# mousecpn/Boosting-R-CNN

Hardware: AMD Instinct MI355X
Metric: images/sec (1333x800) Boosting R-CNN R50-PAFPN inference (higher is better)
Workload: dtype f32; 1 GPU; boosting_rcnn_r50_pafpn_1x_utdac.py inference (model(return_loss=False, rescale=True): device pass + result copy + bbox2result), batch 8 x 3x800x1344 per GPU, f32 MFMA conv stack, 1000 pre-NMS / 256 proposals per image, seeded synthetic weights; global_batch=8, parallelism=dp1

## Files before the change

### boosting-r-cnn_amd/csrc/conv_common.h

```cpp
#pragma once
#include "common.h"

namespace brcnn_conv {

typedef float f32x16 __attribute__((ext_vector_type(16)));
typedef float f32x4 __attribute__((ext_vector_type(4)));
typedef unsigned int u32x4 __attribute__((ext_vector_type(4)));

constexpr int OOB = 0x7fffffff;

constexpr int BK = 32, LDS_STRIDE = 36;

struct ConvParams {
    const float* x;
    const float* w;
    const float* scale;
    const float* shift;
    const float* residual;
    float* y;
    int batch, Cin, Cout, KH, KW, stride, pad;
    int M, K;
    int relu;
    int tiles_m, tiles_n;
    int pitch;
// ... 60 lines not shown
        const int qh = hi / dilate, qw = wi / dilate;
        ok = ok & (qh * dilate == hi) & (qw * dilate == wi);
        hi = qh;
        wi = qw;
    }
}

typedef short brcnn_i16x2 __attribute__((ext_vector_type(2)));
__device__ __forceinline__ float brcnn_relu1(float v) { return __builtin_amdgcn_fmed3f(v, 0.f, __builtin_inff()); }
template <int ET> __device__ __forceinline__ brcnn_f32x2 brcnn_unpk2(unsigned w) {
    brcnn_f32x2 r;
    if constexpr (ET) {
        r.x = brcnn_h2f((unsigned short)(w & 0xffffu));
        r.y = brcnn_h2f((unsigned short)(w >> 16));
    } else {
        r.x = __uint_as_float(w << 16);
        r.y = __uint_as_float(w & 0xffff0000u);
    }
    return r;
}
template <int ET> __device__ __forceinline__ unsigned brcnn_pk2(brcnn_f32x2 v) { return ET ? brcnn_pk2h(v.x, v.y) : brcnn_pk2b(v.x, v.y); }
__device__ __forceinline__ unsigned brcnn_relu_pk(unsigned w, unsigned floor2) {
    const brcnn_i16x2 a = __builtin_bit_cast(brcnn_i16x2, w), f = __builtin_bit_cast(brcnn_i16x2, floor2);
    return __builtin_bit_cast(unsigned, __builtin_elementwise_max(a, f));
}

int conv1x1_stream_try(ConvParams& p, hipStream_t s, int f16);
int conv1x1_stream_set(int mode);
int dispatch_conv_bf16(ConvParams& p, hipStream_t s);
int dispatch_conv_pp_bf16(ConvParams& p, hipStream_t s);
int dispatch_conv_pp128_bf16(ConvParams& p, hipStream_t s);
int sk_plan_pp(ConvParams& p, int slots, int bm, int bn, hipStream_t s);
int sk_plan_pp_f32(ConvParams& p, int slots, int bm, int bn, hipStream_t s);
float* conv_ws_wgrad_slabs(hipStream_t s);
float* wgrad_defer_slabs(hipStream_t s, size_t bytes, int* err);
void wgrad_defer_push(hipStream_t s, float* slab, float* dw, int tiles, int tiles_k, int slices, int group, int Cout, int K,
                      int kind);
unsigned* conv_ws_wgrad_counters(hipStream_t s);
int wgrad_pp_bf16_try(const void* x, const void* dy, void* dw, int batch, int num_segments, const int* heights_host,
                      const int* widths_host, int cin, int cout, int kh, int kw, int stride, int pad, hipStream_t stream,
                      int f16);
int wgrad_pp_set(int v);
bool sk_par_enabled();
int dispatch_conv_pp_f32(ConvParams& p, hipStream_t s);

}
```

### boosting-r-cnn_amd/csrc/conv_igemm.hip

```cpp
#include "conv_common.h"

namespace {
using namespace brcnn_conv;

template <bool FAST, int WM, int NT, bool RES>
__global__ __launch_bounds__(128 * WM, 2) void conv_igemm_f32_kernel(ConvParams p) {
    constexpr int THREADS = 128 * WM;
    constexpr int BM = 64 * WM, BN = 64 * NT;
    constexpr int RPP = THREADS / 8;
    constexpr int AJ = BM / RPP;
    constexpr int BJ = (BN + RPP - 1) / RPP;
    extern __shared__ __attribute__((aligned(16))) float smem[];
    float* As = smem;
    float* Bs = smem + 2 * BM * LDS_STRIDE;

    const int tid = threadIdx.x;
    const int lane = tid & 63, wave = tid >> 6;
    const int wm = wave >> 1, wn = wave & 1;
    const int li = lane & 31, lh = lane >> 5;
    const float* __restrict__ xin = p.x;

    const int nwg = p.tiles_m * p.tiles_n;
    const int tile = xcd_remap(blockIdx.x, nwg);
    const int tile_m = tile / p.tiles_n, tile_n = tile - tile_m * p.tiles_n;
// ... 175 lines not shown
        mfma_group(as, bs, 0);
        mfma_group(as, bs, 1);
        if (more) store_tile(cur ^ 1);
        mfma_group(as, bs, 2);
        mfma_group(as, bs, 3);
        __syncthreads();
        cur ^= 1;
    }

    float* __restrict__ yout = p.y;
#pragma unroll
    for (int tn = 0; tn < NT; tn++) {
        const int co = n0 + wn * 32 * NT + tn * 32 + li;
        const bool cok = co < p.Cout;
        const float sc = (p.scale && cok) ? p.scale[co] : 1.f;
        const float sh = (p.shift && cok) ? p.shift[co] : 0.f;
#pragma unroll
        for (int tm = 0; tm < 2; tm++) {
            const int mb = m0 + wm * 64 + tm * 32 + 4 * lh;
#pragma unroll
            for (int r = 0; r < 16; r++) {
                const int m = mb + (r & 3) + 8 * (r >> 2);
                float v = acc[tm][tn][r];
                if (p.scale) v = v * sc;
                v = v + sh;
                if (RES) v = v + rv[tm][tn][r];
                if (p.relu) v = fmaxf(v, 0.f);
                if (cok && m < p.M) yout[(size_t)m * p.Cout + co] = v;
            }
        }
    }
}

template <int MT, int NT, bool RES>
__global__ __launch_bounds__(256, 2) void conv_igemm_f32_dma_kernel(ConvParams p) {
    constexpr int BM = 64 * MT, BN = 64 * NT;
    constexpr int AG = BM / 8 / 4;
    constexpr int BG = BN / 8 / 4;
    extern __shared__ __attribute__((aligned(16))) float smem[];
    float* As = smem;
    float* Bs = smem + 2 * BM * 32;
    typedef __attribute__((address_space(3))) void* lds_ptr_t;

    const int tid = threadIdx.x;
    const int lane = tid & 63;
    const int wave = __builtin_amdgcn_readfirstlane(tid >> 6);
    const int wm = wave >> 1, wn = wave & 1;
    const int li = lane & 31, lh = lane >> 5;

    const int nwg = p.tiles_m * p.tiles_n;
    const int tile = xcd_remap(blockIdx.x, nwg);
    const int tile_m = tile / p.tiles_n, tile_n = tile - tile_m * p.tiles_n;
    const int m0 = tile_m * BM, n0 = tile_n * BN;

    const __amdgpu_buffer_rsrc_t rsrc_x = __builtin_amdgcn_make_buffer_rsrc((void*)p.x, 0, (int)p.x_bytes, 0x00020000);
    const __amdgpu_buffer_rsrc_t rsrc_w = __builtin_amdgcn_make_buffer_rsrc((void*)p.w, 0, (int)p.w_bytes, 0x00020000);

    const int rg = lane >> 3, pc = lane & 7;
    const bool plain = !p.no_fast && p.KH == 1 && p.KW == 1 && p.stride == 1 && p.pad == 0 && p.nseg == 1 && p.dilate <= 1;
    int a_base[AG], a_hw[AG], a_H[AG], a_W[AG], a_lc[AG];
    int b_off[BG];
#pragma unroll
    for (int j = 0; j < AG; j++) {
        const int r = (wave * AG + j) * 8 + rg;
        a_lc[j] = (pc ^ ((r >> 1) & 7)) * 4;
        const int m = m0 + r;
        if (plain) {
            a_base[j] = m < p.M ? (int)p.seg_xoff[0] + m * p.pitch : -1;
            a_hw[j] = (4096 << 16) | 4096;
            a_H[j] = a_W[j] = 1;
        } else if (m < p.M) {
            int sg = 0;
#pragma unroll
            for (int t = 1; t < BRCNN_MAX_LEVELS; t++)
                if (t < p.nseg && m >= p.seg_m0[t]) sg = t;
            const int ml = m - p.seg_m0[sg];
            const int Ho = p.seg_Ho[sg], Wo = p.seg_Wo[sg];
            a_H[j] = p.seg_H[sg];
            a_W[j] = p.seg_W[sg];
            const int n = ml / (Ho * Wo);
            const int rem = ml - n * (Ho * Wo);
            const int ho = rem / Wo, wo = rem - ho * Wo;
            a_base[j] = (int)p.seg_xoff[sg] + n * a_H[j] * a_W[j] * p.pitch;
            a_hw[j] = ((ho * p.stride - p.pad + 4096) << 16) | (wo * p.stride - p.pad + 4096);
        } else {
            a_base[j] = -1;
            a_hw[j] = 0;
            a_H[j] = a_W[j] = 0;
        }
    }
#pragma unroll
    for (int j = 0; j < BG; j++) {
        const int r = (wave * BG + j) * 8 + rg;
        const int co = n0 + r;
        b_off[j] = (co < p.Cout) ? co * p.K + (pc ^ ((r >> 1) & 7)) * 4 : -1;
    }

    f32x16 acc[MT][NT];
#pragma unroll
    for (int a = 0; a < MT; a++)
#pragma unroll
        for (int b = 0; b < NT; b++)
#pragma unroll
            for (int r = 0; r < 16; r++) acc[a][b][r] = 0.f;

    const int nk = (p.K + BK - 1) / BK;

    int d_k0 = 0, d_ci0 = 0, d_kh = 0, d_kw = 0;
    unsigned a_off4[AG], b_off4[BG];
#pragma unroll
    for (int j = 0; j < AG; j++) a_off4[j] = a_base[j] >= 0 ? (unsigned)(a_base[j] + a_lc[j] + tile_n * p.gstep) * 4u : (unsigned)OOB;
#pragma unroll
    for (int j = 0; j < BG; j++) b_off4[j] = b_off[j] >= 0 ? (unsigned)b_off[j] * 4u : (unsigned)OOB;
    unsigned d_plain = 0;
    auto dma_tile_plain = [&](int buf) {
        const unsigned step = d_plain;
        d_plain += BK * 4;
#pragma unroll
        for (int j = 0; j < AG; j++) {
            float* dst = As + buf * BM * 32 + (wave * AG + j) * 8 * 32;
            __builtin_amdgcn_raw_ptr_buffer_load_lds(rsrc_x, (lds_ptr_t)dst, 16, (int)(a_off4[j] + step), 0, 0, 0);
        }
#pragma unroll
        for (int j = 0; j < BG; j++) {
            float* dst = Bs + buf * BN * 32 + (wave * BG + j) * 8 * 32;
            __builtin_amdgcn_raw_ptr_buffer_load_lds(rsrc_w, (lds_ptr_t)dst, 16, (int)(b_off4[j] + step), 0, 0, 0);
        }
    };
    auto dma_tile = [&](int kt, int buf) {
        (void)kt;
        if (plain) { dma_tile_plain(buf); return; }
        const int ci0 = d_ci0, kh = d_kh, kw = d_kw;
        const int k0 = (kh * p.KW + kw) * p.Cin + ci0;
        (void)d_k0;
        if (++d_kw == p.KW) {
            d_kw = 0;
            if (++d_kh == p.KH) { d_kh = 0; d_ci0 += BK; }
        }
#pragma unroll
        for (int j = 0; j < AG; j++) {
            int hi = (a_hw[j] >> 16) - 4096 + kh;
            int wi = (a_hw[j] & 0xffff) - 4096 + kw;
            bool ok = a_base[j] >= 0;
            if (p.dilate > 1) {
                brcnn_undilate(p.dilate, hi, wi, ok);
            }
            ok = ok & ((unsigned)hi < (unsigned)a_H[j]) & ((unsigned)wi < (unsigned)a_W[j]);
            const int off = ok ? (a_base[j] + (hi * a_W[j] + wi) * p.pitch + ci0 + a_lc[j] + tile_n * p.gstep) * 4 : OOB;
            float* dst = As + buf * BM * 32 + (wave * AG + j) * 8 * 32;
            __builtin_amdgcn_raw_ptr_buffer_load_lds(rsrc_x, (lds_ptr_t)dst, 16, off, 0, 0, 0);
        }
#pragma unroll
        for (int j = 0; j < BG; j++) {
            const int off = (b_off[j] >= 0) ? (b_off[j] + k0) * 4 : OOB;
            float* dst = Bs + buf * BN * 32 + (wave * BG + j) * 8 * 32;
            __builtin_amdgcn_raw_ptr_buffer_load_lds(rsrc_w, (lds_ptr_t)dst, 16, off, 0, 0, 0);
        }
    };

    dma_tile(0, 0);

    const float* __restrict__ res = p.residual;
    const bool vec = (p.Cout & 3) == 0;
    const int vrow = lane >> 3, vcol = (lane & 7) * 4;
    float rv[MT][NT][16];
    const bool full = !p.no_fast && vec && !p.scatter && m0 + BM <= p.M && n0 + BN <= p.Cout;
    const size_t row0 = (size_t)(m0 + wm * 32 * MT + vrow) * p.Cout + n0 + wn * 32 * NT + vcol;
// ... 8 lines not shown
                    for (int it = 0; it < 4; it++) {
                        const float4 q = *reinterpret_cast<const float4*>(rrow + (size_t)(tm * 32 + it * 8) * p.Cout + tn * 32);
                        rv[tm][tn][4 * it + 0] = q.x; rv[tm][tn][4 * it + 1] = q.y;
                        rv[tm][tn][4 * it + 2] = q.z; rv[tm][tn][4 * it + 3] = q.w;
                    }
            return;
        }
#pragma unroll
        for (int tn = 0; tn < NT; tn++) {
#pragma unroll
            for (int tm = 0; tm < MT; tm++) {
                if (vec) {
                    const int co = n0 + wn * 32 * NT + tn * 32 + vcol;
#pragma unroll
                    for (int it = 0; it < 4; it++) {
                        const int m = m0 + wm * 32 * MT + tm * 32 + it * 8 + vrow;
                        float4 q = make_float4(0.f, 0.f, 0.f, 0.f);
                        if (co < p.Cout && m < p.M) q = *reinterpret_cast<const float4*>(res + (size_t)m * p.Cout + co);
                        rv[tm][tn][4 * it + 0] = q.x; rv[tm][tn][4 * it + 1] = q.y;
                        rv[tm][tn][4 * it + 2] = q.z; rv[tm][tn][4 * it + 3] = q.w;
                    }
                } else {
                    const int co = n0 + wn * 32 * NT + tn * 32 + li;
                    const int mb = m0 + wm * 32 * MT + tm * 32 + 4 * lh;
#pragma unroll
                    for (int r = 0; r < 16; r++) {
                        const int m = mb + (r & 3) + 8 * (r >> 2);
                        rv[tm][tn][r] = (co < p.Cout && m < p.M) ? res[(size_t)m * p.Cout + co] : 0.f;
                    }
                }
            }
        }
    };
    asm volatile("s_waitcnt vmcnt(0)" ::: "memory");
    __syncthreads();

    const int sw = (li >> 1) & 7;
    unsigned chb[BK / 8];
#pragma unroll
    for (int kk = 0; kk < BK / 8; kk++) chb[kk] = (unsigned)(((2 * kk + lh) ^ sw) * 16);
    const unsigned a_lane = (unsigned)(size_t)(lds_ptr_t)(As + (wm * 32 * MT + li) * 32);
    const unsigned b_lane = (unsigned)(size_t)(lds_ptr_t)(Bs + (wn * 32 * NT + li) * 32);
    f32x4 av[2][MT], bv[2][NT];
    auto frag_read = [&](int slot, unsigned a_addr, unsigned b_addr) {
        asm volatile("ds_read_b128 %0, %1" : "=v"(av[slot][0]) : "v"(a_addr) : "memory");
        if constexpr (MT == 2)
            asm volatile("ds_read_b128 %0, %1 offset:4096" : "=v"(av[slot][1]) : "v"(a_addr) : "memory");
        asm volatile("ds_read_b128 %0, %1" : "=v"(bv[slot][0]) : "v"(b_addr) : "memory");
        if constexpr (NT == 2)
            asm volatile("ds_read_b128 %0, %1 offset:4096" : "=v"(bv[slot][1]) : "v"(b_addr) : "memory");
    };
    auto frag_wait = [&](int slot) {
        if constexpr (MT == 2 && NT == 2)
            asm volatile("s_waitcnt lgkmcnt(0)" : "+v"(av[slot][0]), "+v"(av[slot][1]), "+v"(bv[slot][0]), "+v"(bv[slot][1]) :: "memory");
        else if constexpr (MT == 2)
            asm volatile("s_waitcnt lgkmcnt(0)" : "+v"(av[slot][0]), "+v"(av[slot][1]), "+v"(bv[slot][0]) :: "memory");
        else if constexpr (NT == 2)
            asm volatile("s_waitcnt lgkmcnt(0)" : "+v"(av[slot][0]), "+v"(bv[slot][0]), "+v"(bv[slot][1]) :: "memory");
        else
            asm volatile("s_waitcnt lgkmcnt(0)" : "+v"(av[slot][0]), "+v"(bv[slot][0]) :: "memory");
    };
    auto compute_tile = [&](int cur, bool prefetch) {
        const unsigned a_cur = a_lane + cur * (BM * 32 * 4);
        const unsigned b_cur = b_lane + cur * (BN * 32 * 4);
        __builtin_amdgcn_s_setprio(1);
        frag_read(0, a_cur + chb[0], b_cur + chb[0]);
        if (prefetch) dma_tile(0, cur ^ 1);
        frag_wait(0);
        __builtin_amdgcn_s_setprio(0);
#pragma unroll
        for (int kk = 0; kk < BK / 8; kk++) {
            const int sl = kk & 1;
            if (kk + 1 < BK / 8) frag_read(sl ^ 1, a_cur + chb[kk + 1], b_cur + chb[kk + 1]);
#pragma unroll
            for (int e = 0; e < 4; e++)
#pragma unroll
                for (int tm = 0; tm < MT; tm++)
#pragma unroll
                    for (int t = 0; t < NT; t++)
                        acc[tm][t] = __builtin_amdgcn_mfma_f32_32x32x2f32(av[sl][tm][e], bv[sl][t][e],
                                                                          acc[tm][t], 0, 0, 0);
            if (kk + 1 < BK / 8) frag_wait(sl ^ 1);
        }
    };
    int cur = 0;
    for (int kt = 0; kt + 1 < nk; kt++) {
        compute_tile(cur, true);
        asm volatile("s_waitcnt vmcnt(0)" ::: "memory");
        __syncthreads();
        cur ^= 1;
    }
    if (RES) load_residual();
    compute_tile(cur, false);

    float* __restrict__ yout = p.y;
    float* slab = (wave < 2 ? As + (cur ^ 1) * BM * 32 : Bs + (cur ^ 1) * BN * 32) + (wave & 1) * 1024;
    if (full) {
        float* __restrict__ yrow = yout + row0;
#pragma unroll
        for (int tn = 0; tn < NT; tn++) {
            const int co = n0 + wn * 32 * NT + tn * 32 + li;
            const float sc = p.scale ? p.scale[co] : 1.f;
            const float sh = p.shift ? p.shift[co] : 0.f;
#pragma unroll
            for (int tm = 0; tm < MT; tm++) {
#pragma unroll
                for (int r = 0; r < 16; r += 2) {
                    const brcnn_f32x2 a = brcnn_f32x2{acc[tm][tn][r], acc[tm][tn][r + 1]} * brcnn_f32x2{sc, sc} + brcnn_f32x2{sh, sh};
                    slab[((r & 3) + 8 * (r >> 2) + 4 * lh) * 32 + li] = a.x;
                    slab[(((r + 1) & 3) + 8 * ((r + 1) >> 2) + 4 * lh) * 32 + li] = a.y;
                }
                __builtin_amdgcn_wave_barrier();
#pragma unroll
                for (int it = 0; it < 4; it++) {
                    float4 v = *reinterpret_cast<const float4*>(slab + (it * 8 + vrow) * 32 + vcol);
                    if (RES) {
                        v.x += rv[tm][tn][4 * it + 0]; v.y += rv[tm][tn][4 * it + 1];
                        v.z += rv[tm][tn][4 * it + 2]; v.w += rv[tm][tn][4 * it + 3];
                    }
                    if (p.relu) {
                        v.x = brcnn_relu1(v.x); v.y = brcnn_relu1(v.y); v.z = brcnn_relu1(v.z); v.w = brcnn_relu1(v.w);
                    }
                    *reinterpret_cast<float4*>(yrow + (size_t)(tm * 32 + it * 8) * p.Cout + tn * 32) = v;
                }
                __builtin_amdgcn_wave_barrier();
            }
// ... 25 lines not shown
                    if (RES) {
                        v.x += rv[tm][tn][4 * it + 0]; v.y += rv[tm][tn][4 * it + 1];
                        v.z += rv[tm][tn][4 * it + 2]; v.w += rv[tm][tn][4 * it + 3];
                    }
                    if (p.relu) {
                        v.x = fmaxf(v.x, 0.f); v.y = fmaxf(v.y, 0.f); v.z = fmaxf(v.z, 0.f); v.w = fmaxf(v.w, 0.f);
                    }
                    if (cv < p.Cout && m < p.M) {
                        const long long ro = out_row_offset(p, m);
                        if (ro >= 0) *reinterpret_cast<float4*>(yout + ro + cv) = v;
                    }
                }
                __builtin_amdgcn_wave_barrier();
            } else {
                const int mb = m0 + wm * 32 * MT + tm * 32 + 4 * lh;
#pragma unroll
                for (int r = 0; r < 16; r++) {
                    const int m = mb + (r & 3) + 8 * (r >> 2);
                    float v = acc[tm][tn][r];
                    if (p.scale) v = v * sc;
                    v = v + sh;
                    if (RES) v = v + rv[tm][tn][r];
                    if (p.relu) v = fmaxf(v, 0.f);
                    if (cok && m < p.M) {
                        const long long ro = out_row_offset(p, m);
                        if (ro >= 0) yout[ro + co] = v;
                    }
                }
            }
        }
    }
}

template <int MT, int NT, bool RES>
int launch_dma(const ConvParams& p, hipStream_t s) {
    const size_t lds = (size_t)2 * (64 * MT + 64 * NT) * 32 * sizeof(float);
    static bool attr_done = false;
    if (!attr_done) {
        BRCNN_HIP_CHECK(hipFuncSetAttribute((const void*)conv_igemm_f32_dma_kernel<MT, NT, RES>,
                                            hipFuncAttributeMaxDynamicSharedMemorySize, (int)lds));
        attr_done = true;
    }
    hipLaunchKernelGGL((conv_igemm_f32_dma_kernel<MT, NT, RES>), dim3(p.tiles_m * p.tiles_n), dim3(256), lds,
                       s, p);
    BRCNN_LAUNCH_CHECK();
    return 0;
}

template <bool FAST, int WM, int NT, bool RES>
int launch_conv(const ConvParams& p, hipStream_t s) {
    const size_t lds = (size_t)2 * (64 * WM + 64 * NT) * LDS_STRIDE * sizeof(float);
    static bool attr_done = false;
    if (!attr_done) {
        BRCNN_HIP_CHECK(hipFuncSetAttribute((const void*)conv_igemm_f32_kernel<FAST, WM, NT, RES>,
                                            hipFuncAttributeMaxDynamicSharedMemorySize, (int)lds));
        attr_done = true;
    }
    hipLaunchKernelGGL((conv_igemm_f32_kernel<FAST, WM, NT, RES>), dim3(p.tiles_m * p.tiles_n),
                       dim3(128 * WM), lds, s, p);
    BRCNN_LAUNCH_CHECK();
    return 0;
}

template <bool FAST, int WM, int NT>
int launch_res(const ConvParams& p, hipStream_t s) {
    return p.residual ? launch_conv<FAST, WM, NT, true>(p, s) : launch_conv<FAST, WM, NT, false>(p, s);
}

int g_use_dma = 1;
int g_force_wm = 0, g_force_nt = 0;

int g_no_fast = 0;
int g_pp_f32_n128 = 1;
int g_pp_f32_mode = 1;

int dispatch_conv(ConvParams& p, hipStream_t s) {
    const bool fast = (p.Cin % 32 == 0);
    if (fast && g_pp_f32_mode && g_force_wm == 0 && g_force_nt == 0 && !p.gstep && (p.Cout % 256) == 0 && p.K >= 256 &&
        p.KH * p.KW <= 32 && !(p.dilate > 1 && p.residual)) {
        const long long t48 = (long long)((p.M + 127) / 128) * (p.Cout / 256);
        p.pp_rows = g_pp_f32_mode >= 128 ? g_pp_f32_mode : 0;
        const bool few = sk_par_enabled() && t48 >= 64 && t48 < 208 && p.K / 32 >= 64 && p.dilate <= 1;
        if (g_pp_f32_mode >= 2 || ((t48 >= 208 || few) && (p.K >= 512 || !p.residual))) return dispatch_conv_pp_f32(p, s);
    }
    if (fast && g_pp_f32_mode && g_pp_f32_n128 && g_force_wm == 0 && g_force_nt == 0 && !p.gstep && (p.Cout % 256) != 0 &&
        (p.Cout % 128) == 0 && p.K >= 256 && p.KH * p.KW <= 32 && !(p.dilate > 1 && p.residual)) {
        const long long t = (long long)((p.M + 255) / 256) * (p.Cout / 128);
        p.pp_rows = 0;
        p.pp_cols = 128;
        if (g_pp_f32_n128 >= 2 || (t >= 208 && p.K >= 1024)) return dispatch_conv_pp_f32(p, s);
        p.pp_cols = 0;
    }
    if (fast && g_use_dma && g_force_wm == 0 && g_force_nt == 0) {
        p.tiles_m = (p.M + 63) / 64;
        p.tiles_n = (p.Cout + 63) / 64;
        return p.residual ? launch_dma<1, 1, true>(p, s) : launch_dma<1, 1, false>(p, s);
    }
    int nt = (fast || p.Cout <= 64) ? 1 : 2;
    if (g_force_nt == 1 || (g_force_nt == 2 && p.Cout > 64)) nt = g_force_nt;
    int wm = 2;
    if (g_force_wm == 4 && fast && nt == 2) wm = 4;
    p.tiles_m = (p.M + 64 * wm - 1) / (64 * wm);
    p.tiles_n = (p.Cout + 64 * nt - 1) / (64 * nt);
    if (!fast) return nt == 1 ? launch_res<false, 2, 1>(p, s) : launch_res<false, 2, 2>(p, s);
    if (wm == 2 && g_use_dma) {
        if (g_force_wm == 1) {
            p.tiles_m = (p.M + 63) / 64;
            p.tiles_n = (p.Cout + 63) / 64;
            return p.residual ? launch_dma<1, 1, true>(p, s) : launch_dma<1, 1, false>(p, s);
        }
        if (nt == 1) return p.residual ? launch_dma<2, 1, true>(p, s) : launch_dma<2, 1, false>(p, s);
        return p.residual ? launch_dma<2, 2, true>(p, s) : launch_dma<2, 2, false>(p, s);
    }
    if (nt == 1) return launch_res<true, 2, 1>(p, s);
    return wm == 4 ? launch_res<true, 4, 2>(p, s) : launch_res<true, 2, 2>(p, s);
}

}

namespace brcnn_conv {
int tuning_get_eight_phase_f32() { return g_pp_f32_mode; }
}

BRCNN_API int brcnn_conv_set_tile(int wm, int nt) {
    if (wm == -1) { g_use_dma = nt; return 0; }
    if (wm == -3) { if (nt < 0 || nt > 2) return BRCNN_EINVAL; g_pp_f32_n128 = nt; return 0; }
    if (wm == -4) { if (nt != 0 && nt != 1) return BRCNN_EINVAL; g_no_fast = nt; return 0; }
    if (wm == -2) { if (nt != 0 && nt != 1 && nt != 2 && nt != 128 && nt != 256) return BRCNN_EINVAL; g_pp_f32_mode = nt; return 0; }
    if ((wm != 0 && wm != 1 && wm != 2 && wm != 4) || nt < 0 || nt > 2) return BRCNN_EINVAL;
    g_force_wm = wm;
    g_force_nt = nt;
    return 0;
}

BRCNN_API int brcnn_conv2d_nhwc(const void* x, const void* w, const float* scale, const float* shift,
                                const void* residual, void* y, int batch, int height, int width,
                                int cin, int cout, int kh, int kw, int stride, int pad, int relu,
                                int dtype, void* stream) {
    const int hs[1] = {height}, ws[1] = {width};
    return brcnn_conv2d_nhwc_multi(x, w, scale, shift, residual, y, batch, 1, hs, ws, cin, cout, kh,
                                   kw, stride, pad, relu, dtype, stream);
}

struct TrainTail {
    void* z_out; const float* mean; const float* var; float eps;
    const void* tail_z; float* partials; int tail_relu;
    const void* tail_mask; void* dres;
};

int brcnn_bn_eval_reduce_launch(const float* partials, int strips, const float* mean, const float* var, float eps,
                                float* dgamma, float* dbeta, int channels, hipStream_t s, int defer);

static int conv_setup_and_launch(const void* x, const void* w, const float* scale, const float* shift,
                                 const void* residual, void* y, int batch, int num_segments,
                                 const int* heights_host, const int* widths_host,
                                 const int* out_heights_host, const int* out_widths_host, int cin,
                                 int cout, int kh, int kw, int stride, int pad, int dilate, int relu,
                                 int dtype, void* stream, int pitch = 0, const int* scatter = nullptr,
                                 const TrainTail* tail = nullptr, int* tiles_m_out = nullptr, int stem2 = 0) {
    if (!x || !w || !y || batch <= 0 || cin <= 0 || cout <= 0 || kh <= 0 || kw <= 0 || stride <= 0 ||
// ... 275 lines not shown
```

### boosting-r-cnn_amd/csrc/conv_igemm_bf16.hip

```cpp
#include <algorithm>
#include <mutex>
#include <vector>
#include "conv_common.h"

namespace {
using namespace brcnn_conv;

typedef __bf16 bf16x8 __attribute__((ext_vector_type(8)));
typedef _Float16 f16x8 __attribute__((ext_vector_type(8)));
typedef __attribute__((address_space(3))) void* lds_ptr_t;
constexpr int BKE = 64;

__device__ __forceinline__ unsigned short f2bf(float v) { return brcnn_f2b(v); }
__device__ __forceinline__ float bf2f(unsigned short h) { return __uint_as_float(((unsigned)h) << 16); }
template <int ET> __device__ __forceinline__ float e2f(unsigned short h) { return ET ? brcnn_h2f(h) : bf2f(h); }
template <int ET> __device__ __forceinline__ unsigned short f2e(float v) { return ET ? brcnn_f2h(v) : f2bf(v); }
template <int ET> __device__ __forceinline__ unsigned pk2e(float lo, float hi) { return ET ? brcnn_pk2h(lo, hi) : brcnn_pk2b(lo, hi); }

template <int MT, int NT, bool RES, bool OUTF32, int WM, int WNW = 2, int ST = 2, int ET = 0, int MODE = 0, bool SK = false>
__global__ __launch_bounds__(64 * WM * WNW, (ST == 2 && MT * NT <= 4 && (WM * WNW == 4 || MT == 1)) ? 2 : 1) void conv_igemm_bf16_dma_kernel(ConvParams p) {
    constexpr int NW = WNW * WM;
    constexpr int BM = 32 * MT * WM, BN = 32 * NT * WNW;
    constexpr int AG = BM / 8 / NW;
    constexpr int BG = BN / 8 / NW;
// ... 825 lines not shown
        }
    }
    if (nslots > SK_MAX_SLOTS) return BRCNN_EINVAL;
    size_t maxlen = 0;
    std::vector<Item> queue[8];
    for (int x = 0; x < 8; x++) {
        std::stable_sort(heads[x].begin(), heads[x].end(), [](const Item& a, const Item& b) { return a.ke - a.kb < b.ke - b.kb; });
        std::stable_sort(wholes[x].begin(), wholes[x].end(), [](const Item& a, const Item& b) { return a.tile < b.tile; });
        std::stable_sort(tails[x].begin(), tails[x].end(), [](const Item& a, const Item& b) { return a.ke - a.kb > b.ke - b.kb; });
        queue[x] = heads[x];
        queue[x].insert(queue[x].end(), wholes[x].begin(), wholes[x].end());
        queue[x].insert(queue[x].end(), tails[x].begin(), tails[x].end());
        if (queue[x].size() > maxlen) maxlen = queue[x].size();
    }
    std::vector<int4> host(maxlen * 8);
    for (size_t loc = 0; loc < maxlen; loc++)
        for (int x = 0; x < 8; x++) {
            int4 v = make_int4(-1, 0, 0, 0);
            if (loc < queue[x].size()) v = make_int4(queue[x][loc].tile, queue[x][loc].kb, queue[x][loc].ke, queue[x][loc].slot);
            host[loc * 8 + x] = v;
        }
    SkTable t = {tiles, nk, slots, (int)(maxlen * 8), nullptr, 0};
    BRCNN_HIP_CHECK(hipMalloc((void**)&t.items, host.size() * sizeof(int4)));
    BRCNN_HIP_CHECK(hipMemcpy(t.items, host.data(), host.size() * sizeof(int4), hipMemcpyHostToDevice));
    if (g_sk_tables.capacity() < 256) g_sk_tables.reserve(256);
    if (g_sk_tables.size() >= 256) { (void)hipFree(t.items); return BRCNN_EINVAL; }
    g_sk_tables.push_back(t);
    *out = &g_sk_tables.back();
    return 0;
}

int sk_table_par(long long tiles, int nk, int slots, const SkTable** out) {
    for (auto& t : g_sk_tables)
        if (t.tiles == tiles && t.nk == nk && t.slots == slots && t.par) { *out = &t; return 0; }
    struct Item { int tile, kb, ke, w; };
    std::vector<Item> storing, finishing;
    const long long iters = tiles * nk;
    std::vector<long long> bound((size_t)slots + 1);
    for (int r = 0; r <= slots; r++) {
        long long b = iters * r / slots;
        const long long rem = b % nk;
        if (rem == 1) b -= 1;
        else if (rem == nk - 1) b += 1;
        bound[r] = b;
    }
    std::vector<int> first_range((size_t)tiles, -1);
    for (int r = 0; r < slots; r++) {
        long long sw = bound[r];
        const long long ew = bound[r + 1];
        while (sw < ew) {
            const long long tile = sw / nk, t0 = tile * nk;
            const long long pe = (ew < t0 + nk) ? ew : t0 + nk;
            const int kb = (int)(sw - t0), ke = (int)(pe - t0);
            if (first_range[tile] < 0) first_range[tile] = r;
            if (ke == nk) {
                const int n_prev = r - first_range[tile];
                if (n_prev > 255) return BRCNN_EINVAL;
                finishing.push_back({(int)tile, kb, ke, r | (n_prev << 16) | (1 << 30)});
            } else {
                storing.push_back({(int)tile, kb, ke, r | (1 << 30)});
            }
            sw = pe;
        }
    }
    auto longer = [](const Item& a, const Item& b) { return a.ke - a.kb > b.ke - b.kb; };
    std::stable_sort(storing.begin(), storing.end(), longer);
    std::stable_sort(finishing.begin(), finishing.end(), longer);
    std::vector<int4> host;
    for (auto& it : storing) host.push_back(make_int4(it.tile, it.kb, it.ke, it.w));
    while (host.size() % 8) host.push_back(make_int4(-1, 0, 0, 0));
    for (auto& it : finishing) host.push_back(make_int4(it.tile, it.kb, it.ke, it.w));
    SkTable t = {tiles, nk, slots, (int)host.size(), nullptr, 1};
    BRCNN_HIP_CHECK(hipMalloc((void**)&t.items, host.size() * sizeof(int4)));
    BRCNN_HIP_CHECK(hipMemcpy(t.items, host.data(), host.size() * sizeof(int4), hipMemcpyHostToDevice));
    if (g_sk_tables.capacity() < 256) g_sk_tables.reserve(256);
    if (g_sk_tables.size() >= 256) { (void)hipFree(t.items); return BRCNN_EINVAL; }
    g_sk_tables.push_back(t);
    *out = &g_sk_tables.back();
    return 0;
}

int g_sk_par = 0;

static int sk_plan(ConvParams& p, int slots, int bm, int bn, hipStream_t s, int min_nk = 0, int bke = BKE, double max_eff = 0.9) {
    p.sk_wgs = 0;
    if (int e = sk_take_error()) return e;
    if (g_sk_mode == 0 || slots <= 0 || slots > SK_MAX_SLOTS) return 0;
    {
        hipStreamCaptureStatus cs = hipStreamCaptureStatusNone;
        if (hipStreamIsCapturing(s, &cs) == hipSuccess && cs != hipStreamCaptureStatusNone) return 0;
    }
    const long long tiles = (long long)p.tiles_m * p.tiles_n;
    const int nk = p.K / bke;
    if (nk < 2 || tiles * nk >= 0x7fffffffLL) return 0;
    if ((size_t)(slots + 8) * bm * bn * sizeof(float) > SK_WS_BYTES) return 0;
    if (tiles < slots) {
        if (min_nk <= 0 || g_sk_par == 0) return 0;
        if (g_sk_par == 1 && (tiles * 5 > (long long)slots * 4 || tiles * nk / slots < min_nk / 2 || tiles * nk / slots < 4)) return 0;
        if (tiles * nk / slots < 2) return 0;
        std::lock_guard<std::mutex> lock(g_sk_mutex);
        SkStream* st = nullptr;
        int rc = sk_stream_state(s, &st);
        if (rc) return rc;
        const SkTable* tab = nullptr;
        rc = sk_table_par(tiles, nk, slots, &tab);
        if (rc) return rc == BRCNN_EINVAL ? 0 : rc;
        if (++st->epoch == 0) st->epoch = 1;
        p.sk_wgs = tab->blocks;
        p.sk_items = tab->items;
        p.sk_ws = st->ws;
        p.sk_flags = st->flags;
        p.sk_epoch = st->epoch;
        p.sk_err = g_sk_err_dev;
        p.sk_spin_limit = g_sk_spin_limit;
        p.sk_drop_publish = g_sk_drop_publish;
        return 0;
    }
    if (g_sk_mode == 1) {
        const double gens = (double)tiles / slots;
        const double eff = gens / (double)(long long)(gens + 0.999999);
        if (min_nk > 0) {
            if (eff >= max_eff || nk < min_nk) return 0;
        } else if (eff >= 0.9 || nk < 32 || bm != 128 || bn != 128) {
            return 0;
        }
    }
    std::lock_guard<std::mutex> lock(g_sk_mutex);
    SkStream* st = nullptr;
    int rc = sk_stream_state(s, &st);
    if (rc) return rc;
    const SkTable* tab = nullptr;
    rc = sk_table(tiles, nk, slots, &tab);
    if (rc) return rc == BRCNN_EINVAL ? 0 : rc;
    if (++st->epoch == 0) st->epoch = 1;
    p.sk_wgs = tab->blocks;
    p.sk_items = tab->items;
    p.sk_ws = st->ws;
    p.sk_flags = st->flags;
    p.sk_epoch = st->epoch;
    p.sk_err = g_sk_err_dev;
    p.sk_spin_limit = g_sk_spin_limit;
    p.sk_drop_publish = g_sk_drop_publish;
    return 0;
}

template <int MT, int NT, bool RES, bool OUTF32, int WM = 2, int WNW = 2, int ST = 2, int ET = 0, int MODE = 0>
int launch(ConvParams& p, hipStream_t s) {
    const size_t lds_stage = (size_t)(32 * MT * WM + 32 * NT * WNW) * 32 * sizeof(float);
    const size_t lds_full = ST * lds_stage;
    const size_t lds_epi = (size_t)WNW * WM * 32 * (32 * NT + 4) * sizeof(float);
    const int nk = p.K / BKE;
    if constexpr (ST == 2 && MT * NT <= 4) {
        static int occ = -1;
        static bool sk_attr = false;
        const size_t lds_sk = lds_full > lds_epi ? lds_full : lds_epi;
        if (!sk_attr) {
            BRCNN_HIP_CHECK(hipFuncSetAttribute((const void*)conv_igemm_bf16_dma_kernel<MT, NT, RES, OUTF32, WM, WNW, ST, ET, MODE, true>,
                                                hipFuncAttributeMaxDynamicSharedMemorySize, (int)lds_sk));
            int n = 0;
            BRCNN_HIP_CHECK(hipOccupancyMaxActiveBlocksPerMultiprocessor(
                &n, (const void*)conv_igemm_bf16_dma_kernel<MT, NT, RES, OUTF32, WM, WNW, ST, ET, MODE, true>, 64 * WM * WNW, lds_sk));
            if (g_num_cus == 0) {
                int dev = 0;
                hipDeviceProp_t prop;
                BRCNN_HIP_CHECK(hipGetDevice(&dev));
                BRCNN_HIP_CHECK(hipGetDeviceProperties(&prop, dev));
                g_num_cus = prop.multiProcessorCount;
            }
            occ = n;
            sk_attr = true;
        }
        const int rc = sk_plan(p, occ * g_num_cus, 32 * MT * WM, 32 * NT * WNW, s);
        if (rc) return rc;
        if (p.sk_wgs > 0) {
            hipLaunchKernelGGL((conv_igemm_bf16_dma_kernel<MT, NT, RES, OUTF32, WM, WNW, ST, ET, MODE, true>), dim3(p.sk_wgs),
// ... 44 lines not shown

int g_pp_mode = 1;
static bool pp_wins(const ConvParams& p) {
    if (g_pp_mode == 0 || p.gstep || (p.Cout % 256) || p.K < 512 || (p.K % 64) || p.KH * p.KW > 32 || p.scatter) return false;
    if (p.tail_z && p.tail_mask) return false;
    const long long t88 = (long long)((p.M + 255) / 256) * (p.Cout / 256);
    return t88 >= 128;
}

int g_pp128_mode = 1;
int g_pp128_min_k = 4096;
int g_pp128_max_t88 = 128;
static bool pp128_ok(const ConvParams& p) {
    return !(p.gstep || (p.Cout % 128) || p.K < 192 || (p.K % 64) || p.KH * p.KW > 32 || p.scatter || (p.tail_z && p.tail_mask));
}
static bool pp128_wins(const ConvParams& p) {
    if (g_pp128_mode == 0 || !pp128_ok(p) || p.K < g_pp128_min_k || p.KH * p.KW < 9) return false;
    const long long tm = (p.M + 255) / 256;
    if ((p.Cout % 256) == 0 && tm * (p.Cout / 256) >= g_pp128_max_t88) return false;
    const long long t84 = tm * (p.Cout / 128);
    return t84 >= 128 && t84 <= 264;
}

int g_bf16_il = 0;
int g_bf16_tile = 0;

}

namespace brcnn_conv {
int sk_plan_pp(ConvParams& p, int slots, int bm, int bn, hipStream_t s) { return sk_plan(p, slots, bm, bn, s, 16); }
bool sk_par_enabled() { return g_sk_par != 0 && g_sk_mode != 0; }
int sk_plan_pp_f32(ConvParams& p, int slots, int bm, int bn, hipStream_t s) { return sk_plan(p, slots, bm, bn, s, 8, 32, 0.97); }

static int dispatch_conv_f16(ConvParams& p, hipStream_t s) {
    p.il = 0;
    if (const int rc = conv1x1_stream_try(p, s, 1)) return rc < 0 ? rc : 0;
    if (p.gstep) return launch2<1, 1, 4, 2, 2, 1>(p, s);
    if (pp128_wins(p)) return dispatch_conv_pp128_bf16(p, s);
    if (pp_wins(p)) return dispatch_conv_pp_bf16(p, s);
    const long long t22 = (long long)((p.M + 127) / 128) * ((p.Cout + 127) / 128);
    const long long t44 = (long long)((p.M + 255) / 256) * ((p.Cout + 255) / 256);
    const bool fill44 = p.Cout >= 256 && p.K >= 1024 && !p.residual && !p.out_f32 && !p.z_out && !p.tail_z && t44 >= 512 &&
                        (double)t44 / (double)(((t44 + 255) / 256) * 256) >= 0.85;
    if (fill44 && p.Cout > 128) return launch2<2, 2, 4, 4, 2, 1>(p, s);
    if (p.Cout <= 64) return launch2<2, 1, 2, 2, 2, 1>(p, s);
    if (t22 < 256) return launch2<1, 1, 2, 2, 2, 1>(p, s);
    const bool sk82 = g_sk_mode == 1 && (p.Cout % 128) == 0 && p.K >= 2048 && t22 >= 512 &&
                      (double)t22 / (double)(((t22 + 511) / 512) * 512) < 0.9;
    if (p.M >= 65536 || sk82) return launch2<1, 2, 4, 2, 2, 1>(p, s);
    if (p.M >= 16384) return launch2<1, 1, 4, 2, 2, 1>(p, s);
    return launch2<2, 1, 2, 2, 2, 1>(p, s);
}

int dispatch_conv_bf16(ConvParams& p, hipStream_t s) {
    if (p.f16) return dispatch_conv_f16(p, s);
    p.il = g_bf16_il;
    if (g_bf16_tile == 0) {
        if (const int rc = conv1x1_stream_try(p, s, 0)) return rc < 0 ? rc : 0;
    }
    if (p.gstep) return launch2<1, 1, 4, 2>(p, s);
    int t = ((p.z_out || p.tail_z) && g_bf16_tile != 8844 && g_bf16_tile != 8842) ? 0 : g_bf16_tile;
    if (t == 0 && pp128_wins(p)) return dispatch_conv_pp128_bf16(p, s);
    if (t == 0 && pp_wins(p)) return dispatch_conv_pp_bf16(p, s);
    if (t == 0) {
        const long long t22 = (long long)((p.M + 127) / 128) * ((p.Cout + 127) / 128);
        const long long t44 = (long long)((p.M + 255) / 256) * ((p.Cout + 255) / 256);
// ... 64 lines not shown
```

Baseline: 331.9 images/sec.

## Add persistent stream-K decomposition for f32 DMA 64x64 conv tiles

Adds a stream-K variant of the f32 DMA implicit-GEMM kernel. Each persistent workgroup walks a contiguous range of (tile, k-block) iterations. Partial accumulators are handed between workgroups through a workspace, guarded by epoch flags and spin-waits. It is enabled by default when the tile count leaves a badly balanced last wave, and is meant to cut tail-wave idle CUs. The cost is extra workspace traffic, spin synchronisation, and the serial dependency between neighbouring workgroups.

```diff
diff --git a/boosting-r-cnn_amd/csrc/conv_common.h b/boosting-r-cnn_amd/csrc/conv_common.h
--- a/boosting-r-cnn_amd/csrc/conv_common.h
+++ b/boosting-r-cnn_amd/csrc/conv_common.h
@@ -116,6 +116,7 @@
 int dispatch_conv_pp128_bf16(ConvParams& p, hipStream_t s);
 int sk_plan_pp(ConvParams& p, int slots, int bm, int bn, hipStream_t s);
 int sk_plan_pp_f32(ConvParams& p, int slots, int bm, int bn, hipStream_t s);
+int sk_plan_f32_tile(ConvParams& p, int per_cu, int cus, hipStream_t s);
 float* conv_ws_wgrad_slabs(hipStream_t s);
 float* wgrad_defer_slabs(hipStream_t s, size_t bytes, int* err);
 void wgrad_defer_push(hipStream_t s, float* slab, float* dw, int tiles, int tiles_k, int slices, int group, int Cout, int K,
diff --git a/boosting-r-cnn_amd/csrc/conv_igemm.hip b/boosting-r-cnn_amd/csrc/conv_igemm.hip
--- a/boosting-r-cnn_amd/csrc/conv_igemm.hip
+++ b/boosting-r-cnn_amd/csrc/conv_igemm.hip
@@ -231,12 +231,12 @@
     }
 }
 
-template <int MT, int NT, bool RES>
-__global__ __launch_bounds__(256, 2) void conv_igemm_f32_dma_kernel(ConvParams p) {
+template <int MT, int NT, bool RES, bool SK>
+__device__ __forceinline__ void conv_f32_dma_item(const ConvParams& p, float* smem, const int tile, const int kb_, const int ke_,
+                                                  const int sk_slot) {
     constexpr int BM = 64 * MT, BN = 64 * NT;
     constexpr int AG = BM / 8 / 4;
     constexpr int BG = BN / 8 / 4;
-    extern __shared__ __attribute__((aligned(16))) float smem[];
     float* As = smem;
     float* Bs = smem + 2 * BM * 32;
     typedef __attribute__((address_space(3))) void* lds_ptr_t;
@@ -247,8 +247,6 @@
     const int wm = wave >> 1, wn = wave & 1;
     const int li = lane & 31, lh = lane >> 5;
 
-    const int nwg = p.tiles_m * p.tiles_n;
-    const int tile = xcd_remap(blockIdx.x, nwg);
     const int tile_m = tile / p.tiles_n, tile_n = tile - tile_m * p.tiles_n;
     const int m0 = tile_m * BM, n0 = tile_n * BN;
 
@@ -304,14 +302,25 @@
             for (int r = 0; r < 16; r++) acc[a][b][r] = 0.f;
 
     const int nk = (p.K + BK - 1) / BK;
-
-    int d_k0 = 0, d_ci0 = 0, d_kh = 0, d_kw = 0;
+    const int kb = SK ? kb_ : 0, ke = SK ? ke_ : nk;
+    const bool finish = !SK || ke == nk;
+
+    int d_ci0 = 0, d_kh = 0, d_kw = 0;
+    if constexpr (SK) {
+        if (kb > 0) {
+            const int T = p.KH * p.KW;
+            const int cc = kb / T, tap = kb - cc * T;
+            d_kh = tap / p.KW;
+            d_kw = tap - d_kh * p.KW;
+            d_ci0 = cc * BK;
+        }
+    }
     unsigned a_off4[AG], b_off4[BG];
 #pragma unroll
     for (int j = 0; j < AG; j++) a_off4[j] = a_base[j] >= 0 ? (unsigned)(a_base[j] + a_lc[j] + tile_n * p.gstep) * 4u : (unsigned)OOB;
 #pragma unroll
     for (int j = 0; j < BG; j++) b_off4[j] = b_off[j] >= 0 ? (unsigned)b_off[j] * 4u : (unsigned)OOB;
-    unsigned d_plain = 0;
+    unsigned d_plain = (unsigned)kb * (BK * 4);
     auto dma_tile_plain = [&](int buf) {
         const unsigned step = d_plain;
         d_plain += BK * 4;
@@ -331,7 +340,6 @@
         if (plain) { dma_tile_plain(buf); return; }
         const int ci0 = d_ci0, kh = d_kh, kw = d_kw;
         const int k0 = (kh * p.KW + kw) * p.Cin + ci0;
-        (void)d_k0;
         if (++d_kw == p.KW) {
             d_kw = 0;
             if (++d_kh == p.KH) { d_kh = 0; d_ci0 += BK; }
@@ -406,6 +414,31 @@
             }
         }
     };
+    if constexpr (SK) {
+        if (kb > 0) {
+            if (tid == 0) {
+                int spins = 0;
+                while (__hip_atomic_load(p.sk_flags + sk_slot, __ATOMIC_RELAXED, __HIP_MEMORY_SCOPE_AGENT) != p.sk_epoch &&
+                       ++spins < p.sk_spin_limit)
+                    __builtin_amdgcn_s_sleep(4);
+                if (spins >= p.sk_spin_limit)
+                    __hip_atomic_store(p.sk_err, p.sk_epoch | 0x80000000u, __ATOMIC_RELAXED, __HIP_MEMORY_SCOPE_SYSTEM);
+                __builtin_amdgcn_fence(__ATOMIC_ACQUIRE, "agent");
+            }
+            __syncthreads();
+            const f32x4* src = reinterpret_cast<const f32x4*>(p.sk_ws) + (size_t)sk_slot * (BM * BN / 4) + wave * 64 + lane;
+#pragma unroll
+            for (int a = 0; a < MT; a++)
+#pragma unroll
+                for (int b = 0; b < NT; b++)
+#pragma unroll
+                    for (int g = 0; g < 4; g++) {
+                        const f32x4 v = src[((a * NT + b) * 4 + g) * 256];
+                        acc[a][b][4 * g + 0] = v.x; acc[a][b][4 * g + 1] = v.y;
+                        acc[a][b][4 * g + 2] = v.z; acc[a][b][4 * g + 3] = v.w;
+                    }
+        }
+    }
     asm volatile("s_waitcnt vmcnt(0)" ::: "memory");
     __syncthreads();
 
@@ -458,14 +491,40 @@
         }
     };
     int cur = 0;
-    for (int kt = 0; kt + 1 < nk; kt++) {
+    for (int kt = kb; kt + 1 < ke; kt++) {
         compute_tile(cur, true);
         asm volatile("s_waitcnt vmcnt(0)" ::: "memory");
         __syncthreads();
         cur ^= 1;
     }
-    if (RES) load_residual();
+    if (RES && finish) load_residual();
     compute_tile(cur, false);
+
+    if constexpr (SK) {
+        if (!finish) {
+            f32x4* dst = reinterpret_cast<f32x4*>(p.sk_ws) + (size_t)sk_slot * (BM * BN / 4) + wave * 64 + lane;
+#pragma unroll
+            for (int a = 0; a < MT; a++)
+#pragma unroll
+                for (int b = 0; b < NT; b++)
+#pragma unroll
+                    for (int g = 0; g < 4; g++) {
+                        f32x4 v;
+                        v.x = acc[a][b][4 * g + 0]; v.y = acc[a][b][4 * g + 1];
+                        v.z = acc[a][b][4 * g + 2]; v.w = acc[a][b][4 * g + 3];
+                        dst[((a * NT + b) * 4 + g) * 256] = v;
+                    }
+            asm volatile("s_waitcnt vmcnt(0)" ::: "memory");
+            __syncthreads();
+            if (tid == 0) {
+                __builtin_amdgcn_fence(__ATOMIC_RELEASE, "agent");
+                asm volatile("s_waitcnt vmcnt(0)" ::: "memory");
+                if (!p.sk_drop_publish)
+                    __hip_atomic_store(p.sk_flags + sk_slot, p.sk_epoch, __ATOMIC_RELAXED, __HIP_MEMORY_SCOPE_AGENT);
+            }
+            return;
+        }
+    }
 
     float* __restrict__ yout = p.y;
     float* slab = (wave < 2 ? As + (cur ^ 1) * BM * 32 : Bs + (cur ^ 1) * BN * 32) + (wave & 1) * 1024;
@@ -557,9 +616,73 @@
     }
 }
 
+template <int MT, int NT, bool RES, bool SK = false>
+__global__ __launch_bounds__(256, 2) void conv_igemm_f32_dma_kernel(ConvParams p) {
+    extern __shared__ __attribute__((aligned(16))) float smem[];
+    if constexpr (SK) {
+        const int4 range = p.sk_items[blockIdx.x];
+        const int first = __builtin_amdgcn_readfirstlane(range.x), count = __builtin_amdgcn_readfirstlane(range.y);
+        for (int i = 0; i < count; i++) {
+            if (i > 0) __syncthreads();
+            const int4 item = p.sk_items[first + i];
+            conv_f32_dma_item<MT, NT, RES, true>(p, smem, __builtin_amdgcn_readfirstlane(item.x),
+                                                 __builtin_amdgcn_readfirstlane(item.y), __builtin_amdgcn_readfirstlane(item.z),
+                                                 __builtin_amdgcn_readfirstlane(item.w));
+        }
+    } else {
+        conv_f32_dma_item<MT, NT, RES, false>(p, smem, xcd_remap(blockIdx.x, p.tiles_m * p.tiles_n), 0, 0, 0);
+    }
+}
+
+static bool f32_tile_sk_wins(const ConvParams& p, int per_cu, int cus) {
+    const long long tiles = (long long)p.tiles_m * p.tiles_n;
+    if (tiles >= (long long)per_cu * cus || tiles < 2LL * cus || p.K / BK < 64) return false;
+    const long long busiest = (tiles + cus - 1) / cus * cus;
+    return busiest * 5 >= tiles * 6;
+}
+
+int g_f32_tile_sk = 1;
+int g_f32_tile_sk_launches = 0;
+int g_f32_tile_sk_wgs = 0;
+int g_f32_tile_sk_per_cu = 0;
+int g_f32_num_cus = 0;
+
 template <int MT, int NT, bool RES>
-int launch_dma(const ConvParams& p, hipStream_t s) {
+int launch_dma(ConvParams& p, hipStream_t s, int persistent = 0) {
     const size_t lds = (size_t)2 * (64 * MT + 64 * NT) * 32 * sizeof(float);
+    if constexpr (MT == 1 && NT == 1) {
+        if (persistent) {
+            static int occ = -1;
+            if (occ < 0) {
+                BRCNN_HIP_CHECK(hipFuncSetAttribute((const void*)conv_igemm_f32_dma_kernel<1, 1, RES, true>,
+                                                    hipFuncAttributeMaxDynamicSharedMemorySize, (int)lds));
+                int n = 0;
+                BRCNN_HIP_CHECK(hipOccupancyMaxActiveBlocksPerMultiprocessor(
+                    &n, (const void*)conv_igemm_f32_dma_kernel<1, 1, RES, true>, 256, lds));
+                if (g_f32_num_cus == 0) {
+                    int dev = 0;
+                    hipDeviceProp_t prop;
+                    BRCNN_HIP_CHECK(hipGetDevice(&dev));
+                    BRCNN_HIP_CHECK(hipGetDeviceProperties(&prop, dev));
+                    g_f32_num_cus = prop.multiProcessorCount;
+                }
+                occ = n;
+            }
+            const int per_cu = g_f32_tile_sk_per_cu > 0 && g_f32_tile_sk_per_cu < occ ? g_f32_tile_sk_per_cu : occ;
+            p.sk_wgs = 0;
+            if (persistent >= 2 || f32_tile_sk_wins(p, per_cu, g_f32_num_cus)) {
+                const int rc = sk_plan_f32_tile(p, per_cu, g_f32_num_cus, s);
+                if (rc) return rc;
+            }
+            if (p.sk_wgs > 0) {
+                hipLaunchKernelGGL((conv_igemm_f32_dma_kernel<1, 1, RES, true>), dim3(p.sk_wgs), dim3(256), lds, s, p);
+                BRCNN_LAUNCH_CHECK();
+                g_f32_tile_sk_launches = (g_f32_tile_sk_launches + 1) & 0x7fffffff;
+                g_f32_tile_sk_wgs = p.sk_wgs;
+                return 0;
+            }
+        }
+    }
     static bool attr_done = false;
     if (!attr_done) {
         BRCNN_HIP_CHECK(hipFuncSetAttribute((const void*)conv_igemm_f32_dma_kernel<MT, NT, RES>,
@@ -619,7 +742,8 @@
     if (fast && g_use_dma && g_force_wm == 0 && g_force_nt == 0) {
         p.tiles_m = (p.M + 63) / 64;
         p.tiles_n = (p.Cout + 63) / 64;
-        return p.residual ? launch_dma<1, 1, true>(p, s) : launch_dma<1, 1, false>(p, s);
+        const int sk = (!p.scatter && !p.gstep && p.dilate <= 1) ? g_f32_tile_sk : 0;
+        return p.residual ? launch_dma<1, 1, true>(p, s, sk) : launch_dma<1, 1, false>(p, s, sk);
     }
     int nt = (fast || p.Cout <= 64) ? 1 : 2;
     if (g_force_nt == 1 || (g_force_nt == 2 && p.Cout > 64)) nt = g_force_nt;
@@ -651,6 +775,9 @@
     if (wm == -1) { g_use_dma = nt; return 0; }
     if (wm == -3) { if (nt < 0 || nt > 2) return BRCNN_EINVAL; g_pp_f32_n128 = nt; return 0; }
     if (wm == -4) { if (nt != 0 && nt != 1) return BRCNN_EINVAL; g_no_fast = nt; return 0; }
+    if (wm == -5) { if (nt < 0 || nt > 2) return BRCNN_EINVAL; g_f32_tile_sk = nt; return 0; }
+    if (wm == -7) { if (nt < 0 || nt > 8) return BRCNN_EINVAL; g_f32_tile_sk_per_cu = nt; return 0; }
+    if (wm == -6) return nt == 0 ? g_f32_tile_sk_launches : nt == 1 ? g_f32_tile_sk_wgs : BRCNN_EINVAL;
     if (wm == -2) { if (nt != 0 && nt != 1 && nt != 2 && nt != 128 && nt != 256) return BRCNN_EINVAL; g_pp_f32_mode = nt; return 0; }
     if ((wm != 0 && wm != 1 && wm != 2 && wm != 4) || nt < 0 || nt > 2) return BRCNN_EINVAL;
     g_force_wm = wm;
diff --git a/boosting-r-cnn_amd/csrc/conv_igemm_bf16.hip b/boosting-r-cnn_amd/csrc/conv_igemm_bf16.hip
--- a/boosting-r-cnn_amd/csrc/conv_igemm_bf16.hip
+++ b/boosting-r-cnn_amd/csrc/conv_igemm_bf16.hip
@@ -881,7 +881,7 @@
 
 int sk_table_par(long long tiles, int nk, int slots, const SkTable** out) {
     for (auto& t : g_sk_tables)
-        if (t.tiles == tiles && t.nk == nk && t.slots == slots && t.par) { *out = &t; return 0; }
+        if (t.tiles == tiles && t.nk == nk && t.slots == slots && t.par == 1) { *out = &t; return 0; }
     struct Item { int tile, kb, ke, w; };
     std::vector<Item> storing, finishing;
     const long long iters = tiles * nk;
@@ -929,16 +929,60 @@
     return 0;
 }
 
+int sk_table_ranges(long long tiles, int nk, int slots, const SkTable** out) {
+    for (auto& t : g_sk_tables)
+        if (t.tiles == tiles && t.nk == nk && t.slots == slots && t.par == 2) { *out = &t; return 0; }
+    const long long iters = tiles * nk, q = iters / slots, r = iters % slots;
+    if (q < nk) return BRCNN_EINVAL;
+    std::vector<int4> index((size_t)slots), items;
+    const int cq = slots >> 3, cr = slots & 7;
+    for (int b = 0; b < slots; b++) {
+        const int x = b & 7, loc = b >> 3;
+        const int w = ((x < cr) ? x * (cq + 1) : cr * (cq + 1) + (x - cr) * cq) + loc;
+        const long long sw = q * w + (w < r ? w : r), ew = sw + q + (w < r ? 1 : 0);
+        const long long t_first = sw / nk, t_end = ew / nk;
+        const int kb = (int)(sw - t_first * nk), ke = (int)(ew - t_end * nk);
+        const int first = slots + (int)items.size();
+        if (ke > 0) items.push_back(make_int4((int)t_end, 0, ke, w));
+        for (long long t = t_first + (kb > 0 ? 1 : 0); t < t_end; t++) items.push_back(make_int4((int)t, 0, nk, 0));
+        if (kb > 0) items.push_back(make_int4((int)t_first, kb, nk, w - 1));
+        index[(size_t)b] = make_int4(first, slots + (int)items.size() - first, 0, 0);
+    }
+    index.insert(index.end(), items.begin(), items.end());
+    SkTable t = {tiles, nk, slots, slots, nullptr, 2};
+    BRCNN_HIP_CHECK(hipMalloc((void**)&t.items, index.size() * sizeof(int4)));
+    BRCNN_HIP_CHECK(hipMemcpy(t.items, index.data(), index.size() * sizeof(int4), hipMemcpyHostToDevice));
+    if (g_sk_tables.capacity() < 256) g_sk_tables.reserve(256);
+    if (g_sk_tables.size() >= 256) { (void)hipFree(t.items); return BRCNN_EINVAL; }
+    g_sk_tables.push_back(t);
+    *out = &g_sk_tables.back();
+    return 0;
+}
+
 int g_sk_par = 0;
+
+static bool sk_capturing(hipStream_t s) {
+    hipStreamCaptureStatus cs = hipStreamCaptureStatusNone;
+    return hipStreamIsCapturing(s, &cs) == hipSuccess && cs != hipStreamCaptureStatusNone;
+}
+
+static void sk_fill(ConvParams& p, SkStream& st, const SkTable& tab) {
+    if (++st.epoch == 0) st.epoch = 1;
+    p.sk_wgs = tab.blocks;
+    p.sk_items = tab.items;
+    p.sk_ws = st.ws;
+    p.sk_flags = st.flags;
+    p.sk_epoch = st.epoch;
+    p.sk_err = g_sk_err_dev;
+    p.sk_spin_limit = g_sk_spin_limit;
+    p.sk_drop_publish = g_sk_drop_publish;
+}
 
 static int sk_plan(ConvParams& p, int slots, int bm, int bn, hipStream_t s, int min_nk = 0, int bke = BKE, double max_eff = 0.9) {
     p.sk_wgs = 0;
     if (int e = sk_take_error()) return e;
     if (g_sk_mode == 0 || slots <= 0 || slots > SK_MAX_SLOTS) return 0;
-    {
-        hipStreamCaptureStatus cs = hipStreamCaptureStatusNone;
-        if (hipStreamIsCapturing(s, &cs) == hipSuccess && cs != hipStreamCaptureStatusNone) return 0;
-    }
+    if (sk_capturing(s)) return 0;
     const long long tiles = (long long)p.tiles_m * p.tiles_n;
     const int nk = p.K / bke;
     if (nk < 2 || tiles * nk >= 0x7fffffffLL) return 0;
@@ -954,15 +998,7 @@
         const SkTable* tab = nullptr;
         rc = sk_table_par(tiles, nk, slots, &tab);
         if (rc) return rc == BRCNN_EINVAL ? 0 : rc;
-        if (++st->epoch == 0) st->epoch = 1;
-        p.sk_wgs = tab->blocks;
-        p.sk_items = tab->items;
-        p.sk_ws = st->ws;
-        p.sk_flags = st->flags;
-        p.sk_epoch = st->epoch;
-        p.sk_err = g_sk_err_dev;
-        p.sk_spin_limit = g_sk_spin_limit;
-        p.sk_drop_publish = g_sk_drop_publish;
+        sk_fill(p, *st, *tab);
         return 0;
     }
     if (g_sk_mode == 1) {
@@ -981,15 +1017,7 @@
     const SkTable* tab = nullptr;
     rc = sk_table(tiles, nk, slots, &tab);
     if (rc) return rc == BRCNN_EINVAL ? 0 : rc;
-    if (++st->epoch == 0) st->epoch = 1;
-    p.sk_wgs = tab->blocks;
-    p.sk_items = tab->items;
-    p.sk_ws = st->ws;
-    p.sk_flags = st->flags;
-    p.sk_epoch = st->epoch;
-    p.sk_err = g_sk_err_dev;
-    p.sk_spin_limit = g_sk_spin_limit;
-    p.sk_drop_publish = g_sk_drop_publish;
+    sk_fill(p, *st, *tab);
     return 0;
 }
 
@@ -1100,6 +1128,30 @@
 bool sk_par_enabled() { return g_sk_par != 0 && g_sk_mode != 0; }
 int sk_plan_pp_f32(ConvParams& p, int slots, int bm, int bn, hipStream_t s) { return sk_plan(p, slots, bm, bn, s, 8, 32, 0.97); }
 
+int sk_plan_f32_tile(ConvParams& p, int per_cu, int cus, hipStream_t s) {
+    p.sk_wgs = 0;
+    if (int e = sk_take_error()) return e;
+    if (g_sk_mode == 0 || per_cu <= 0 || cus <= 0) return 0;
+    if ((long long)p.tiles_m * p.tiles_n < (long long)per_cu * cus) per_cu = (int)((long long)p.tiles_m * p.tiles_n / cus);
+    if (per_cu < 2) return 0;
+    const int slots = per_cu * cus;
+    if (slots > SK_MAX_SLOTS) return 0;
+    if (sk_capturing(s)) return 0;
+    const long long tiles = (long long)p.tiles_m * p.tiles_n;
+    const int nk = p.K / 32;
+    if (nk < 2 || (p.K % 32) || tiles < slots || tiles * nk >= 0x7fffffffLL) return 0;
+    if ((size_t)slots * 64 * 64 * sizeof(float) > SK_WS_BYTES) return 0;
+    std::lock_guard<std::mutex> lock(g_sk_mutex);
+    SkStream* st = nullptr;
+    int rc = sk_stream_state(s, &st);
+    if (rc) return rc;
+    const SkTable* tab = nullptr;
+    rc = sk_table_ranges(tiles, nk, slots, &tab);
+    if (rc) return rc == BRCNN_EINVAL ? 0 : rc;
+    sk_fill(p, *st, *tab);
+    return 0;
+}
+
 static int dispatch_conv_f16(ConvParams& p, hipStream_t s) {
     p.il = 0;
     if (const int rc = conv1x1_stream_try(p, s, 1)) return rc < 0 ? rc : 0;
```

New measurement: 337.7 images/sec, median of 6. 1.02x the previous value.
